# augustgw/early-exit-transformer

Hardware: AMD Instinct MI355X
Metric: mel-frames/sec encoder forward (all exits) + summed per-exit CTC loss, d_model=256 12-layer (higher is better)
Workload: dtype fp16x3 (hi/lo-split fp16 MFMA operands, three products per GEMM, fp32 accumulate; v_mfma_f32_16x16x32_f16); 1 GPU; early_conformer ctc 12-layer d_model=256 (6 exits x 2), batch 64/GPU, mel [80 x 1027] -> T'=256, log-normal synthetic mel, random-init weights (BASELINE.json configs[1]); global_batch=64, mel_frames=1027, parallelism=dp1 (utterance-batch shards), precision_mode=f16x3

## Files before the change

early_exit_transformer_amd/csrc/eec_blocks.h:

```cpp
#pragma once
#include "eec_kernels.h"

namespace eec {

constexpr int kLinThreads = 512;
template <int D>
constexpr int kLinLds = 2 * Geo<D>::kAPlane;
#ifndef EEC_LPF
#define EEC_LPF 4
#endif
constexpr int kLPF = EEC_LPF;

constexpr int kQkvStageLd = 80, kQkvStageLdV = 144, kQkvStageBytes = 64 * kQkvStageLd;
static_assert(32 * kQkvStageLdV <= kQkvStageBytes, "V^T staging fits the Q / K staging area");
constexpr int kQkvFragLd = 1056;
static_assert(4 * kQkvFragLd <= kQkvStageBytes && (kQkvFragLd / 2) % 16 == 0, "fragment-major V^T staging");
__device__ __forceinline__ int vt_perm(int t) {
  return (t & ~12) | ((t & 4) << 1) | ((t & 8) >> 1);
}

template <int MT, int NT>
__device__ __forceinline__ void acc_init_bias(f32x16 (&acc)[MT][NT], const float* __restrict__ bias_n0, float scale = 1.0f) {
  const int hh = lane_id() >> 5;
#pragma unroll
  for (int nt = 0; nt < NT; ++nt)
#pragma unroll
    for (int g = 0; g < 4; ++g) {
      const float4 bb = *(const float4*)(bias_n0 + 32 * nt + 8 * g + 4 * hh);
#pragma unroll
      for (int mt = 0; mt < MT; ++mt) {
        acc[mt][nt][4 * g + 0] = bb.x * scale;
        acc[mt][nt][4 * g + 1] = bb.y * scale;
        acc[mt][nt][4 * g + 2] = bb.z * scale;
        acc[mt][nt][4 * g + 3] = bb.w * scale;
      }
    }
}

template <int NP, int MT, int NT>
__device__ __forceinline__ void acc_init_bias_np(f32x16 (&acc)[MT][NT], const float* __restrict__ bias_n0, float scale = 1.0f) {
  if constexpr (kMfma16For<NP>) {
    const int lane = lane_id(), hh = lane >> 5, u = (lane >> 4) & 1;
#pragma unroll
    for (int nt = 0; nt < NT; ++nt)
#pragma unroll
      for (int ra = 0; ra < 2; ++ra) {
        const float4 bb = *(const float4*)(bias_n0 + 32 * nt + 16 * ra + 8 * hh + 4 * u);
#pragma unroll
        for (int mt = 0; mt < MT; ++mt)
#pragma unroll
          for (int cb = 0; cb < 2; ++cb) {
            acc[mt][nt][4 * (2 * ra + cb) + 0] = bb.x * scale;
            acc[mt][nt][4 * (2 * ra + cb) + 1] = bb.y * scale;
            acc[mt][nt][4 * (2 * ra + cb) + 2] = bb.z * scale;
            acc[mt][nt][4 * (2 * ra + cb) + 3] = bb.w * scale;
          }
      }
  } else {
    acc_init_bias<MT, NT>(acc, bias_n0, scale);
  }
}

template <int KS>
__device__ __forceinline__ const uint4* wfrag_lane(const uint4* wp, int nt) {
  return wp + (size_t)nt * KS * 128 + lane_id();
}

constexpr int kProjNWB = 2;
template <int NP, int PF, int NT>
struct ProjStream {
  WRing<(NP == 8 ? 1 : NP), PF, NT> r;
  WGroupF8<NT> wg[NP == 8 ? kProjNWB : 1];
};
struct WMat {
  const uint4* wp;
  const uint4* wf8;
};
template <int D, int NP, int PF, int NT>
__device__ __forceinline__ void proj_fill(ProjStream<NP, PF, NT>& st, const WMat& w, int t0) {
  constexpr int KS = D / 16, NG = D / 64;
  if constexpr (NP == 8) {
    const uint4* rec = w.wf8 + (size_t)t0 * NG * kF8Rec + lane_id();
    ring_fill_f8<PF, NT>(st.r, rec, (size_t)NG * kF8Rec);
#pragma unroll
    for (int g = 0; g < kProjNWB; ++g) f8_group_load<NT>(st.wg[g], rec + (size_t)g * kF8Rec, (size_t)NG * kF8Rec);
  } else {
    ring_fill<NP, PF, NT>(st.r, wfrag_lane<KS>(w.wp, t0), (size_t)KS * 128, KS);
  }
}
template <int D, int NP, int PF, int NT, int MT>
__device__ __forceinline__ void proj_gemm(f32x16 (&acc)[MT][NT], const char* smem, ProjStream<NP, PF, NT>& st, const WMat& w, int t0,
                                          int row_stride_mul = 1) {
  using G = Geo<D>;
  constexpr int KS = D / 16, NG = D / 64;
  const int lane = lane_id(), hh = lane >> 5;
  const char* a_lane = smem + (lane & 31) * G::kALd + hh * 16;
  if constexpr (NP == 8) {
    const char* a8_lane = smem + G::kAPlane + (lane & 31) * G::kA8Ld + hh * 32;
    const uint4* rec = w.wf8 + (size_t)t0 * NG * kF8Rec + lane;
    gemm_ring_f8<NG, NT, true, PF, NoSide, 0, kProjNWB, MT>(acc, a_lane, G::kALd, a8_lane, G::kA8Ld, rec,
                                                                                                    (size_t)NG * kF8Rec, st.r, st.wg);
  } else {
    gemm_ring<NP, KS, NT, true, PF, NoSide, 0, MT, !kMfma16For<NP>, true>(acc, a_lane, G::kALd, G::kAPlane, wfrag_lane<KS>(w.wp, t0), (size_t)KS * 128, st.r);
  }
  (void)row_stride_mul;
}

template <int D, int NP>
__device__ __forceinline__ void qkv_body(char* smem, const QkvArgs& a, int row0, ProjStream<NP, kLPF, Geo<D>::kNW>& rq, char* stage = nullptr) {
  using G = Geo<D>;
  constexpr int MT = G::kMT, NW = G::kNW;
  const int lane = lane_id(), w = wave_id(), hh = lane >> 5;
  const int dh = D / a.H;
  const bool fast = D == 256 && stage != nullptr && dh == 32 && a.Tq % G::kRows == 0 && a.Tp == a.Tq;
  char* const stg = stage ? stage + w * kQkvStageBytes : nullptr;
  [[maybe_unused]] auto store_rows_fast = [&](const f32x16 (&acc)[MT][NW], float scale, half_t* p_hi, half_t* p_lo, size_t off) {
    h4 lo4[MT][4];
#pragma unroll
    for (int mt = 0; mt < MT; ++mt)
#pragma unroll
      for (int g = 0; g < 4; ++g) {
        h4 o;
#pragma unroll
        for (int i = 0; i < 4; ++i) {
          const float v = acc[mt][0][4 * g + i] * scale;
          o[i] = to_half_sat(v);
          lo4[mt][g][i] = (half_t)(v - (float)o[i]);
        }
        *(h4*)(stg + (mt * 32 + (lane & 31)) * kQkvStageLd + (8 * g + 4 * hh) * 2) = o;
      }
    asm volatile("" ::: "memory");
    auto tile_out = [&](half_t* dstp) {
      if (a.vt_frag) {
#pragma unroll
        for (int k = 0; k < 4; ++k)
          *(uint4*)(dstp + off + k * 512 + lane * 8) = *(const uint4*)(stg + ((k >> 1) * 32 + (lane & 31)) * kQkvStageLd + (k & 1) * 32 + hh * 16);
      } else {
#pragma unroll
        for (int k = 0; k < 4; ++k) {
          const int row = (lane >> 2) + 16 * k;
          *(uint4*)(dstp + off + (size_t)row * 32 + (lane & 3) * 8) = *(const uint4*)(stg + row * kQkvStageLd + (lane & 3) * 16);
        }
      }
    };
    tile_out(p_hi);
    asm volatile("" ::: "memory");
    if (p_lo) {
#pragma unroll
      for (int mt = 0; mt < MT; ++mt)
#pragma unroll
        for (int g = 0; g < 4; ++g) *(h4*)(stg + (mt * 32 + (lane & 31)) * kQkvStageLd + (8 * g + 4 * hh) * 2) = lo4[mt][g];
      asm volatile("" ::: "memory");
      tile_out(p_lo);
      asm volatile("" ::: "memory");
    }
  };
  const WMat wm{a.wp, a.wf8};
  ProjStream<NP, kLPF, NW> rk;
  int rb[MT], rt[MT];
  bool ok[MT];
#pragma unroll
  for (int mt = 0; mt < MT; ++mt) {
    const int row = row0 + mt * 32 + (lane & 31);
    ok[mt] = row < a.M;
    rb[mt] = row / a.Tq;
    rt[mt] = row - rb[mt] * a.Tq;
  }
  const int t0 = NW * w;
  constexpr int TQ = D / 32;
  int hd[NW], d0[NW];
#pragma unroll
  for (int j = 0; j < NW; ++j) {
    const int n0 = 32 * (t0 + j);
    hd[j] = n0 / dh;
    d0[j] = n0 - hd[j] * dh + 4 * hh;
  }

  f32x16 acc[MT][NW];
  proj_fill<D, NP, kLPF, NW>(rk, wm, TQ + t0);
  acc_init_bias_np<NP, MT, NW>(acc, a.bias + 32 * t0);
  proj_gemm<D, NP, kLPF, NW, MT>(acc, smem, rq, wm, t0);
  proj_fill<D, NP, kLPF, NW>(rq, wm, 2 * TQ + t0);
  if (fast) {
    if constexpr (D == 256) {
      const int b0 = row0 / a.Tq, tt0 = row0 - b0 * a.Tq;
      store_rows_fast(acc, kLog2e * rsqrtf((float)dh), a.q, a.q_lo, ((size_t)(b0 * a.H + w) * a.Tp + tt0) * 32);
    }
  } else {
    const float scale = kLog2e * rsqrtf((float)dh);
#pragma unroll
    for (int mt = 0; mt < MT; ++mt)
      if (ok[mt]) {
#pragma unroll
        for (int j = 0; j < NW; ++j) {
          const size_t qoff = ((size_t)(rb[mt] * a.H + hd[j]) * a.Tp + rt[mt]) * dh + d0[j];
          half_t* dst = a.q + qoff;
#pragma unroll
          for (int g = 0; g < 4; ++g) {
            h4 o, ol;
#pragma unroll
            for (int i = 0; i < 4; ++i) {
              const float v = acc[mt][j][4 * g + i] * scale;
              o[i] = to_half_sat(v);
              ol[i] = (half_t)(v - (float)o[i]);
            }
            *(h4*)(dst + 8 * g) = o;
            if (a.q_lo) *(h4*)(a.q_lo + qoff + 8 * g) = ol;
          }
        }
      }
  }
  acc_init_bias_np<NP, MT, NW>(acc, a.bias + D + 32 * t0);
  proj_gemm<D, NP, kLPF, NW, MT>(acc, smem, rk, wm, TQ + t0);
  if (fast) {
    if constexpr (D == 256) {
      const int b0 = row0 / a.Tq, tt0 = row0 - b0 * a.Tq;
      store_rows_fast(acc, 1.0f, a.k, a.k_lo, ((size_t)(b0 * a.H + w) * a.Tp + tt0) * 32);
    }
  } else
#pragma unroll
  for (int mt = 0; mt < MT; ++mt)
    if (ok[mt]) {
#pragma unroll
      for (int j = 0; j < NW; ++j) {
        const size_t koff = ((size_t)(rb[mt] * a.H + hd[j]) * a.Tp + rt[mt]) * dh + d0[j];
        half_t* dst = a.k + koff;
#pragma unroll
        for (int g = 0; g < 4; ++g) {
          h4 o, ol;
#pragma unroll
          for (int i = 0; i < 4; ++i) {
            const float v = acc[mt][j][4 * g + i];
            o[i] = to_half_sat(v);
            ol[i] = (half_t)(v - (float)o[i]);
          }
          *(h4*)(dst + 8 * g) = o;
          if (a.k_lo) *(h4*)(a.k_lo + koff + 8 * g) = ol;
        }
      }
    }
  acc_init_bias_np<NP, MT, NW>(acc, a.bias + 2 * D + 32 * t0);
  proj_gemm<D, NP, kLPF, NW, MT>(acc, smem, rq, wm, 2 * TQ + t0);
  if (fast) {
    if constexpr (D == 256) {
      const int b0 = row0 / a.Tq, tt0 = row0 - b0 * a.Tq;
      const size_t vbase = ((size_t)(b0 * a.H + w) * 32) * a.Tp + tt0;
      const int dstride = a.vt_frag ? 16 : kQkvStageLdV;
      int sbase[MT];
#pragma unroll
      for (int mt = 0; mt < MT; ++mt) {
        const int tcol = vt_perm(mt * 32 + (lane & 31));
        sbase[mt] = a.vt_frag ? ((tcol >> 5) * 2 + ((tcol >> 4) & 1)) * kQkvFragLd + ((tcol >> 3) & 1) * (kQkvFragLd / 2) + (tcol & 7) * 2 : tcol * 2;
      }
      auto plane = [&](half_t* dstp, bool lo_plane) {
#pragma unroll
        for (int mt = 0; mt < MT; ++mt)
#pragma unroll
          for (int g = 0; g < 4; ++g)
#pragma unroll
            for (int i = 0; i < 4; ++i) {
              const float v = acc[mt][0][4 * g + i];
              const half_t hi = to_half_sat(v);
              *(half_t*)(stg + sbase[mt] + (8 * g + 4 * hh + i) * dstride) = lo_plane ? (half_t)(v - (float)hi) : hi;
            }
        asm volatile("" ::: "memory");
        if (a.vt_frag) {
          half_t* const fb = dstp + (size_t)(b0 * a.H + w) * 32 * a.Tp + (size_t)(tt0 >> 5) * 1024;
#pragma unroll
          for (int k = 0; k < 4; ++k)
            *(uint4*)(fb + k * 512 + lane * 8) = *(const uint4*)(stg + k * kQkvFragLd + (lane >> 5) * (kQkvFragLd / 2) + (lane & 31) * 16);
        } else {
#pragma unroll
          for (int k = 0; k < 4; ++k) {
            const int d = (lane >> 3) + 8 * k;
            *(uint4*)(dstp + vbase + (size_t)d * a.Tp + (lane & 7) * 8) = *(const uint4*)(stg + d * kQkvStageLdV + (lane & 7) * 16);
          }
        }
        asm volatile("" ::: "memory");
      };
      plane(a.vt, false);
      if (a.vt_lo) plane(a.vt_lo, true);
    }
  } else
#pragma unroll
  for (int mt = 0; mt < MT; ++mt)
    if (ok[mt]) {
#pragma unroll
      for (int j = 0; j < NW; ++j) {
        const size_t voff = ((size_t)(rb[mt] * a.H + hd[j]) * dh + d0[j]) * a.Tp + vt_perm(rt[mt]);
        half_t* dst = a.vt + voff;
#pragma unroll
        for (int g = 0; g < 4; ++g)
#pragma unroll
          for (int i = 0; i < 4; ++i) {
            const float v = acc[mt][j][4 * g + i];
            const half_t hi = to_half_sat(v);
            *(dst + (size_t)(8 * g + i) * a.Tp) = hi;
            if (a.vt_lo) {
              half_t* const lo = a.vt_lo + voff + (size_t)(8 * g + i) * a.Tp;
              *lo = (half_t)(v - (float)hi);
            }
          }
      }
    }
}

constexpr int kDwTaps = 31;
constexpr int kDwHalo = (kDwTaps - 1) / 2;
constexpr int kDwFrames = 16;
constexpr int kDwWin = kDwFrames + kDwTaps - 1;
constexpr int kDPF = 4;
template <int D>
struct DwGeo {
  using G = Geo<D>;
  static constexpr bool kTapsLds = D == 256;
  static constexpr int kGRows = G::kRows + kDwTaps - 1;
  static constexpr int kGLd = D * 2;
  static constexpr int kLds = 2 * G::kAPlane + kGRows * kGLd + (kTapsLds ? kDwTaps * D * 4 : 0);
  static_assert((D / 2) * (G::kRows / kDwFrames) == 512, "thread = 2 channels x 16 frames");
};

template <int D, int NP>
__device__ __forceinline__ void dw_front(char* smem, const DwArgs& d, int M, int row0) {
  using G = Geo<D>;
  using DG = DwGeo<D>;
  constexpr int kGRows = DG::kGRows, kGLd = DG::kGLd;
  char* lds_g = smem + 2 * G::kAPlane;
  float* lds_w = (float*)(lds_g + kGRows * kGLd);
  const int Tq = d.Tq;
  const int c = (threadIdx.x % (D / 2)) * 2, tg = threadIdx.x / (D / 2);
  typedef float f32x2 __attribute__((ext_vector_type(2)));
  [[maybe_unused]] f32x2 taps[DG::kTapsLds ? 1 : kDwTaps];
  {
    constexpr int PPR = D / 8;
    constexpr int GIT = (kGRows * PPR + 511) / 512, WIT = DG::kTapsLds ? (kDwTaps * D / 4 + 511) / 512 : 1;
    uint4 gv[GIT];
    [[maybe_unused]] float4 wv[WIT];
#pragma unroll
    for (int it = 0; it < GIT; ++it) {
      const int p = it * 512 + threadIdx.x, rl = p / PPR, c16 = p % PPR, row = row0 - kDwHalo + rl;
      gv[it] = make_uint4(0, 0, 0, 0);
      if (rl < kGRows && row >= 0 && row < M) gv[it] = *(const uint4*)(d.g + (size_t)row * D + c16 * 8);
    }
    if constexpr (DG::kTapsLds) {
#pragma unroll
      for (int it = 0; it < WIT; ++it) {
        const int p = it * 512 + threadIdx.x;
        wv[it] = make_float4(0.f, 0.f, 0.f, 0.f);
        if (p < kDwTaps * D / 4) wv[it] = ((const float4*)d.wfold)[p];
      }
    } else {
      static_range<0, kDwTaps>([&](auto jt) { taps[decltype(jt)::value] = *(const f32x2*)(d.wfold + decltype(jt)::value * D + c); });
    }
    __builtin_amdgcn_sched_barrier(0);
#pragma unroll
    for (int it = 0; it < GIT; ++it) {
      const int p = it * 512 + threadIdx.x, rl = p / PPR, c16 = p % PPR;
// ... 159 lines not shown
```

early_exit_transformer_amd/csrc/ffn.hip:

```cpp
#ifdef EEC_FFN_TRAIN_BWD
#define EEC_OPERAND_BF16 1
#endif
#if defined(EEC_FFN_TRAIN) || defined(EEC_FFN_TRAIN_BWD)
#define EEC_MFMA16_NP1 1
#endif
#include "eec_blocks.h"
#include "eec_drop.h"

namespace eec {

constexpr int kFfnThreads = 512;
constexpr int kFC = 128;
constexpr int kHLd = (kFC + 8) * 2;
template <int D>
struct FfnGeo {
  using G = Geo<D>;
  static constexpr int kHPlane = G::kRows * kHLd;
  static constexpr int kNT2 = D / 128;
  static constexpr int kLds = 2 * G::kAPlane + (4 * kHPlane > G::kETile ? 4 * kHPlane : G::kETile);
};
#ifndef EEC_TR_NT
#define EEC_TR_NT 1
#endif
#if defined(EEC_FFN_TRAIN_BWD) && !defined(EEC_PF1_NP3)
// ... 87 lines not shown
};

template <int D, int NPN, bool HAS_RES>
__device__ __forceinline__ void chain_rowpass(char* smem, const char* lds_e, float* __restrict__ x, RowV<Geo<D>::kQ> (&xr)[Geo<D>::kRPW],
                                              int row0, int M, float scale, const float* __restrict__ fin_g,
                                              const float* __restrict__ fin_b, float* __restrict__ tap,
                                              const float* __restrict__ nln_g, const float* __restrict__ nln_b,
                                              int lane = lane_id(), int w = wave_id()) {
  using G = Geo<D>;
  constexpr int RPW = G::kRPW, Q = G::kQ;
  RowV<Q> v[RPW];
#pragma unroll
  for (int i = 0; i < RPW; ++i) {
    v[i] = HAS_RES ? xr[i] : zero_row<Q>();
#pragma unroll
    for (int q = 0; q < Q; ++q) {
      const float4 e = *(const float4*)(lds_e + (w * RPW + i) * G::kELd + (q * 256 + lane * 4) * 4);
      v[i].p[q].x += scale * e.x;
      v[i].p[q].y += scale * e.y;
      v[i].p[q].z += scale * e.z;
      v[i].p[q].w += scale * e.w;
    }
  }
  if (fin_g) layer_norm_rows<D, RPW>(v, load_row<D>(fin_g, lane), load_row<D>(fin_b, lane));
#pragma unroll
  for (int i = 0; i < RPW; ++i) {
    const int row = row0 + w * RPW + i;
    if (row < M) {
      store_row<D>(x + (size_t)row * D, v[i], lane);
      if (tap) store_row<D>(tap + (size_t)row * D, v[i], lane);
    }
  }
  if constexpr (NPN != 0) {
    layer_norm_rows<D, RPW>(v, load_row<D>(nln_g, lane), load_row<D>(nln_b, lane));
    rows_to_planes<D, NPN, RPW>(smem, v, w * RPW, row0, M, true, lane);
  }
}

template <int D, int NP, int ACT, int FNP, int QNP, int NS, int TR = 0>
#ifndef EEC_FFN_MINWAVES
#define EEC_FFN_MINWAVES 2
#endif
__global__ __launch_bounds__(kFfnThreads, EEC_FFN_MINWAVES) void ffn_chain_kernel(ChainArgs a) {
  static_assert(!TR || (FNP == 0 && QNP == 0 && NS == 1 && ACT == 2 && NP != 8), "TR: one plain stage");
  static_assert(TR || ACT != 2, "ACT = 2 is the training variant's");
  static_assert((TR == 2) == (EEC_OPERAND_BF16 != 0), "the backward variant (and only it) runs on bf16 operands");
  using G = Geo<D>;
  using FG = FfnGeo<D>;
  constexpr int MT = G::kMT, NW = G::kNW, KS = G::kKS, RPW = G::kRPW, NT2 = FG::kNT2;
  constexpr int kALd = G::kALd, kAPlane = G::kAPlane, kA8Ld = G::kA8Ld, kHPlane = FG::kHPlane;
  constexpr size_t nts = (size_t)KS * 128;
  extern __shared__ __attribute__((aligned(16))) char smem[];
  constexpr int kPF1 = FfnPf<D, NP>::P1, kPF2 = FfnPf<D, NP>::P2;
  constexpr int NH = (NP == 8 && NT2 > 2) ? NT2 / 2 : 1, NTP = NT2 / NH;
  const int lane = lane_id(), w = wave_id();
  const int hh = lane >> 5, wl = w & 3;
  const int w_s = wave_id_sgpr();
  const int wl_s = w_s & 3;
  const bool is_producer = w < 4;
  const int row0 = row_tile_index() * G::kRows;
  const int M = a.M, F = a.F;
  float* __restrict__ x = a.x;
  char* lds_h = smem + 2 * kAPlane;
  char* lds_e = lds_h;
  const char* a_lane = smem + (lane & 31) * kALd + hh * 16;

  const int nft = F / 32;
  const int nchunk = (nft + 3) / 4;
  const int ks2_total = F / 16;
#ifndef EEC_SKEW
#define EEC_SKEW 56
#endif
#ifndef EEC_WARM_SLOTS
#define EEC_WARM_SLOTS 4
#endif
  auto phys = [&](int c) { return c >= nchunk ? c - nchunk : c; };
  const size_t w2_nt_stride = (size_t)ks2_total * 128;

#ifdef EEC_TIMELINE
  int tl_idx = 0;
#endif
  TL_STAMP();
#if EEC_SKEW > 0
  for (int i = 0; i < (int)((blockIdx.x >> 3) & 3); ++i) __builtin_amdgcn_s_sleep(EEC_SKEW);
#endif
  constexpr int RNP = NP == 8 ? 1 : NP;
  constexpr bool Q16 = kMfma16For<NP>;
  auto run = [&](auto prod_tag) {
  constexpr bool producer = decltype(prod_tag)::value;
  [[maybe_unused]] const eect::DropState ds_act(eect::Drop{TR ? a.tr.p : 0.0f, a.tr.seed, a.tr.site_act});
  WRing<RNP, kPF1, 1> r1;
  WRing<RNP, kPF2, NTP> r2;
  WGroupF8<1> wg1[kNW1];
  WGroupF8<NTP> wg2[kNW2];
  const size_t w2f8_nt = (size_t)(F / 64) * kF8Rec;
  auto w1f8_lane = [&](const WPtrs& W, int ft) { return W.w1f8 + (size_t)ft * (D / 64) * kF8Rec + lane; };
  auto w2f8_lane = [&](const WPtrs& W, int c, int h = 0) {
    return W.w2f8 + ((size_t)(NT2 * wl + NTP * h) * (F / 64) + 2 * c) * kF8Rec + lane;
  };
  auto fill1 = [&](const WPtrs& W, int ft) {
    if constexpr (NP == 8) {
      ring_fill_f8<kPF1, 1>(r1, w1f8_lane(W, ft), 0);
#pragma unroll
      for (int g = 0; g < kNW1; ++g) f8_group_load<1>(wg1[g], w1f8_lane(W, ft) + (size_t)g * kF8Rec, 0);
    } else {
      ring_fill<RNP, kPF1, 1>(r1, W.w1p + (size_t)ft * nts + lane, 0, KS);
// ... 4 lines not shown
      ring_fill_f8<kPF2, NTP>(r2, w2f8_lane(W, c), w2f8_nt);
#pragma unroll
      for (int g = 0; g < kNW2; ++g) f8_group_load<NTP>(wg2[g], w2f8_lane(W, c) + (size_t)g * kF8Rec, w2f8_nt);
    } else {
      ring_fill<RNP, kPF2, NTP>(r2, W.w2p + ((size_t)(NT2 * wl) * ks2_total + c * (kFC / 16)) * 128 + lane, w2_nt_stride,
                             min(kFC / 16, ks2_total - c * (kFC / 16)));
    }
  };
  auto start_streams = [&](const WPtrs& W) {
    if constexpr (producer) {
      if (wl < nft) fill1(W, phys(0) * 4 + wl);
    } else {
      fill2(W, phys(0));
    }
  };
#define EEC_STAGE_FIELD(si, f) ((si) == 0 ? a.st[0].f : a.st[1].f)
  auto wptrs = [&](int si) {
    return WPtrs{EEC_STAGE_FIELD(si, w1p), EEC_STAGE_FIELD(si, w2p), EEC_STAGE_FIELD(si, w1f8), EEC_STAGE_FIELD(si, w2f8)};
  };

  unsigned sink_front = 0;
  if constexpr (FNP != 0) {
    ProjStream<FNP, kDPF, NW> rp;
    proj_fill<D, FNP, kDPF, NW>(rp, WMat{a.pw2.wp, a.pw2.wf8}, NW * w);
#if EEC_WARM_SLOTS > 0
    {
      const WPtrs W0 = wptrs(0);
      const size_t wbytes = NP == 8 ? (size_t)(F / 32) * (D / 64) * kF8Rec * 16 : (size_t)F * D * 2 * (NP == 3 ? 2 : 1);
      unsigned t = 0;
#pragma unroll
      for (int j = 0; j < 2; ++j) {
        t ^= touch_share(NP == 8 ? (const void*)W0.w1f8 : (const void*)W0.w1p, wbytes, wl, j);
        t ^= touch_share(NP == 8 ? (const void*)W0.w2f8 : (const void*)W0.w2p, wbytes, wl, j);
      }
      sink_front = t;
    }
#endif
    TL_STAMP();
    dw_front<D, FNP>(smem, a.dw, M, row0);
    TL_STAMP();
    RowV<G::kQ> xr[RPW];
#pragma unroll
    for (int i = 0; i < RPW; ++i) {
      const int row = row0 + w * RPW + i;
      xr[i] = zero_row<G::kQ>();
      if (row < M) xr[i] = load_row<D>(x + (size_t)row * D, lane);
    }
    __builtin_amdgcn_sched_barrier(0);
    __syncthreads();
    TL_STAMP();
    f32x16 accp[MT][NW];
    pw2_gemm<D, FNP>(accp, smem, a.pw2, rp);
    TL_STAMP();
    start_streams(wptrs(0));
    acc_swapped_to_etile<MT, NW>(lds_e, G::kELd, accp, 32 * NW * w);
    __syncthreads();
    TL_STAMP();
    chain_rowpass<D, NP, true>(smem, lds_e, x, xr, row0, M, 1.0f, nullptr, nullptr, nullptr, a.st[0].ln_g, a.st[0].ln_b);
  } else {
    const WPtrs W0 = wptrs(0);
    if constexpr (TR == 2) {
      const eect::DropState ds_res(eect::Drop{a.tr.p, a.tr.seed, a.tr.site_res});
      const float rsc = a.st[0].res_scale;
      RowV<G::kQ> v[RPW];
#pragma unroll
      for (int i = 0; i < RPW; ++i) {
        const int row = row0 + w * RPW + i;
        v[i] = zero_row<G::kQ>();
        if (row < M) v[i] = load_row<D>(x + (size_t)row * D, lane);
      }
      __builtin_amdgcn_sched_barrier(0);
      start_streams(W0);
      if (a.tr.pl_x) {
        constexpr int Q = G::kQ;
        const RowV<Q> gam = load_row<D>(a.tr.pl_g, lane);
        RowV<Q> xh[RPW];
        float rsd[RPW], c1[RPW], c2[RPW];
        RowV<Q> dgs = zero_row<Q>(), dbs = zero_row<Q>();
#pragma unroll
        for (int i = 0; i < RPW; ++i) {
          const int row = row0 + w * RPW + i;
          const bool ok = row < M;
          const float mu = ok ? a.tr.pl_mean[row] : 0.0f;
          rsd[i] = ok ? a.tr.pl_rstd[row] : 0.0f;
          xh[i] = ok ? load_row<D>(a.tr.pl_x + (size_t)row * D, lane) : zero_row<Q>();
          c1[i] = 0.0f, c2[i] = 0.0f;
#pragma unroll
          for (int q = 0; q < Q; ++q) {
            float4& h = xh[i].p[q];
            h.x = (h.x - mu) * rsd[i], h.y = (h.y - mu) * rsd[i], h.z = (h.z - mu) * rsd[i], h.w = (h.w - mu) * rsd[i];
            const float4 ev = v[i].p[q], gq = gam.p[q];
            const float tx = ev.x * gq.x, ty = ev.y * gq.y, tz = ev.z * gq.z, tw = ev.w * gq.w;
            c1[i] += tx + ty + tz + tw;
            c2[i] += tx * h.x + ty * h.y + tz * h.z + tw * h.w;
            dgs.p[q].x += ev.x * h.x, dgs.p[q].y += ev.y * h.y, dgs.p[q].z += ev.z * h.z, dgs.p[q].w += ev.w * h.w;
            dbs.p[q].x += ev.x, dbs.p[q].y += ev.y, dbs.p[q].z += ev.z, dbs.p[q].w += ev.w;
          }
        }
        wave_sum_n<RPW>(c1);
        wave_sum_n<RPW>(c2);
#pragma unroll
        for (int i = 0; i < RPW; ++i) {
          const int row = row0 + w * RPW + i;
          const float m1 = c1[i] * (1.0f / D), m2 = c2[i] * (1.0f / D);
#pragma unroll
          for (int q = 0; q < Q; ++q) {
// ... 5 lines not shown
          }
          if (row < M) store_row<D>(x + (size_t)row * D, v[i], lane);
        }
        float* pw = a.tr.pl_part + ((size_t)blockIdx.x * 8 + w) * 2 * D;
#pragma unroll
        for (int q = 0; q < Q; ++q) {
          *(float4*)(pw + q * 256 + lane * 4) = dgs.p[q];
          *(float4*)(pw + D + q * 256 + lane * 4) = dbs.p[q];
        }
      }
#pragma unroll
      for (int i = 0; i < RPW; ++i) {
        const int row = row0 + w * RPW + i;
#pragma unroll
        for (int q = 0; q < G::kQ; ++q) {
          float m[4];
          ds_res.mul4((size_t)row * D + q * 256 + lane * 4, m);
          v[i].p[q].x *= rsc * m[0], v[i].p[q].y *= rsc * m[1], v[i].p[q].z *= rsc * m[2], v[i].p[q].w *= rsc * m[3];
        }
        if (row < M) store_row<D>(a.tr.ln + (size_t)row * D, v[i], lane);
      }
      rows_to_planes<D, NP, RPW>(smem, v, w * RPW, row0, M, false);
    } else if constexpr (TR == 1) {
      const RowV<G::kQ> lg = load_row<D>(a.st[0].ln_g, lane), lb = load_row<D>(a.st[0].ln_b, lane);
      RowV<G::kQ> v[RPW];
#pragma unroll
      for (int i = 0; i < RPW; ++i) {
        const int row = row0 + w * RPW + i;
        v[i] = zero_row<G::kQ>();
        if (row < M) v[i] = load_row<D>(x + (size_t)row * D, lane);
      }
      __builtin_amdgcn_sched_barrier(0);
      start_streams(W0);
      float mu[RPW], rs[RPW];
      layer_norm_rows<D, RPW>(v, lg, lb, mu, rs);
#pragma unroll
      for (int i = 0; i < RPW; ++i) {
        const int row = row0 + w * RPW + i;
        if (row < M) {
          store_row<D>(a.tr.ln + (size_t)row * D, v[i], lane);
          if (lane == 0) a.tr.mean[row] = mu[i], a.tr.rstd[row] = rs[i];
        }
      }
      rows_to_planes<D, NP, RPW>(smem, v, w * RPW, row0, M, true);
    } else {
      rows_f32_to_planes<D, NP, true>(smem, x, row0, M, a.st[0].ln_g, a.st[0].ln_b, [&]() { start_streams(W0); });
    }
  }
  TL_STAMP();
  __syncthreads();
  TL_STAMP();

  [[maybe_unused]] ProjStream<(QNP ? QNP : 1), kLPF, NW> rq;
  unsigned sink = 0;
  const int nslots = nchunk + 2;
  f32x16 acc2c[NH][MT][NTP];
  static_range<0, NS>([&](auto si_tag) {
    constexpr int si = decltype(si_tag)::value;
    const WPtrs W = wptrs(si);
    const float* __restrict__ b1s = EEC_STAGE_FIELD(si, b1);
    if constexpr (producer) {
      [[maybe_unused]] f32x16 preq[TR == 2 ? MT : 1];
      [[maybe_unused]] auto request_pre = [&](int hcol0) {
#pragma unroll
        for (int mt = 0; mt < MT; ++mt)
#pragma unroll
          for (int g = 0; g < 4; ++g) {
            const int frame = Q16 ? mt * 32 + 16 * (g & 1) + (lane & 15) : mt * 32 + (lane & 31);
            const int hid = Q16 ? wl * 32 + 16 * (g >> 1) + 8 * hh + 4 * ((lane >> 4) & 1) : wl * 32 + 4 * hh + g * 8;
            const int row = min(row0 + frame, M - 1);
            const f32x4 v = __builtin_nontemporal_load((const f32x4*)(a.tr.pre + (size_t)row * F + hcol0 + hid));
            preq[mt][4 * g] = v[0], preq[mt][4 * g + 1] = v[1], preq[mt][4 * g + 2] = v[2], preq[mt][4 * g + 3] = v[3];
          }
      };
      auto silu_pair = [&](const f32x16 (&acc)[MT][1], char* hb, int step, h2& keep_hi, h2& keep_lo, [[maybe_unused]] int hcol0 = 0) {
        const int mt = step >> 3, q = step & 7;
        const float u0 = acc[mt][0][2 * q], u1 = acc[mt][0][2 * q + 1];
        if constexpr (TR == 2) {
          const float x0 = preq[mt][2 * q], x1 = preq[mt][2 * q + 1];
          const float sg0 = __builtin_amdgcn_rcpf(1.0f + __builtin_amdgcn_exp2f(-kLog2e * x0));
          const float sg1 = __builtin_amdgcn_rcpf(1.0f + __builtin_amdgcn_exp2f(-kLog2e * x1));
          const float t0 = u0 * sg0 * (1.0f + x0 * (1.0f - sg0)), t1 = u1 * sg1 * (1.0f + x1 * (1.0f - sg1));
          if ((q & 1) == 0) {
            keep_hi = __builtin_bit_cast(h2, t0);
            keep_lo = __builtin_bit_cast(h2, t1);
            return;
          }
          const int g = q >> 1;
          const int frame = Q16 ? mt * 32 + 16 * (g & 1) + (lane & 15) : mt * 32 + (lane & 31);
          const int hid = Q16 ? wl * 32 + 16 * (g >> 1) + 8 * hh + 4 * ((lane >> 4) & 1) : wl * 32 + 4 * hh + g * 8;
          const int row = row0 + frame;
          const size_t idx = (size_t)row * F + hcol0 + hid;
          float m[4];
          ds_act.mul4(idx, m);
          const float d0 = __builtin_bit_cast(float, keep_hi) * m[0], d1 = __builtin_bit_cast(float, keep_lo) * m[1], d2 = t0 * m[2], d3 = t1 * m[3];
          if (row < M) tape_store4(a.tr.act + idx, d0, d1, d2, d3);
          constexpr int SNPT = NP == 1 ? 1 : 3;
          const hl2_t sa = split2<SNPT>(d0, d1), sb = split2<SNPT>(d2, d3);
          char* dst = hb + frame * kHLd + hid * 2;
          h4 hi, lo;
          hi.xy = sa.hi, hi.zw = sb.hi, lo.xy = sa.lo, lo.zw = sb.lo;
          *(h4*)dst = hi;
          if (NP == 3) *(h4*)(dst + kHPlane) = lo;
          return;
        }
        if constexpr (TR == 1) {
// ... 127 lines not shown
      }
    } else {
#pragma unroll
      for (int h = 0; h < NH; ++h) zero_acc(acc2c[h]);
#if EEC_WARM_SLOTS > 0
      unsigned warm[4] = {0u, 0u, 0u, 0u};
#endif
      for (int s = 0; s < nslots; ++s) {
#if EEC_WARM_SLOTS > 0
        if (s == nslots - EEC_WARM_SLOTS) {
          const int lane_t = fresh_lane();
          if constexpr (si + 1 < NS) {
            const WPtrs Wn = wptrs(si + 1);
            const size_t wbytes = NP == 8 ? (size_t)(F / 32) * (D / 64) * kF8Rec * 16 : (size_t)F * D * 2 * (NP == 3 ? 2 : 1);
#pragma unroll
            for (int j = 0; j < 2; ++j) {
              warm[j] = touch_share(NP == 8 ? (const void*)Wn.w1f8 : (const void*)Wn.w1p, wbytes, wl_s, j, lane_t);
              warm[2 + j] = touch_share(NP == 8 ? (const void*)Wn.w2f8 : (const void*)Wn.w2p, wbytes, wl_s, j, lane_t);
            }
          } else if constexpr (QNP != 0) {
            warm[0] = QNP == 8 ? touch_share(a.qkv.wf8, (size_t)(3 * D / 32) * (D / 64) * kF8Rec * 16, wl_s, 0, lane_t)
                               : touch_share(a.qkv.wp, (size_t)3 * D * D * 2 * (QNP == 3 ? 2 : 1), wl_s, 0, lane_t);
          }
        }
#endif
        if (s >= 2) {
          const int cl = s - 2, c = phys(cl);
          const char* h_lane = lds_h + (cl & 1) * 2 * kHPlane + (lane & 31) * kHLd + hh * 16;
          const int ks2 = min(kFC / 16, ks2_total - c * (kFC / 16));
          const uint4* w2_lane = W.w2p + ((size_t)(NT2 * wl) * ks2_total + c * (kFC / 16)) * 128 + lane;
          if constexpr (NP == 8) {
            const char* h8_lane = lds_h + (cl & 1) * 2 * kHPlane + kHPlane + (lane & 31) * kH8Ld + hh * 32;
            if constexpr (NH == 1) {
              gemm_ring_f8<2, NTP, false, kPF2, NoSide, 0, kNW2, MT>(acc2c[0], h_lane, kHLd, h8_lane, kH8Ld, w2f8_lane(W, c), w2f8_nt, r2, wg2);
            } else {
#pragma unroll
              for (int h = 0; h < NH; ++h) {
                const uint4* next = h + 1 < NH ? w2f8_lane(W, c, h + 1) : (cl + 1 < nchunk ? w2f8_lane(W, phys(cl + 1), 0) : nullptr);
                gemm_ring_f8<2, NTP, false, kPF2, NoSide, 0, kNW2, MT, true>(acc2c[h], h_lane, kHLd, h8_lane, kH8Ld, w2f8_lane(W, c, h), w2f8_nt, r2, wg2, NoSide(), next);
              }
            }
          } else if (ks2 == kFC / 16) {
            gemm_ring<RNP, kFC / 16, NTP, false, kPF2, NoSide, 0, MT, !Q16, !Q16>(acc2c[0], h_lane, kHLd, kHPlane, w2_lane, w2_nt_stride, r2);
          } else {
            gemm_plain<RNP, NTP, false, MT, !Q16, !Q16>(acc2c[0], h_lane, kHLd, kHPlane, w2_lane, w2_nt_stride, ks2);
          }
          if (NH == 1 && cl + 1 < nchunk) fill2(W, phys(cl + 1));
        }
        TL_STAMP();
        __syncthreads();
        TL_STAMP();
      }
#if EEC_WARM_SLOTS > 0
      sink ^= warm[0] ^ warm[1] ^ warm[2] ^ warm[3];
#endif
    }
    const int lane_e = fresh_lane(), w_e = w_s;
    RowV<G::kQ> xr[RPW];
#pragma unroll
    for (int i = 0; i < RPW; ++i) {
      const int row = row0 + w_e * RPW + i;
      xr[i] = zero_row<G::kQ>();
      if (TR != 2 && row < M) xr[i] = load_row<D>(x + (size_t)row * D, lane_e);
    }
    __builtin_amdgcn_sched_barrier(0);
    constexpr bool more = si + 1 < NS;
    TL_STAMP();
    if constexpr (!producer) {
      if constexpr (Q16) {
#pragma unroll
        for (int h = 0; h < NH; ++h) accs_q_to_std<MT, NTP>(acc2c[h]);
      }
#pragma unroll
      for (int h = 0; h < NH; ++h)
        acc_to_etile<MT, NTP>(lds_e, G::kELd, acc2c[h], wl_s * 32 * NT2 + h * 32 * NTP, EEC_STAGE_FIELD(si, b2), lane_e);
    }
    TL_STAMP();
    if constexpr (more) {
      start_streams(wptrs(1));
    } else if constexpr (QNP != 0) {
      proj_fill<D, QNP, kLPF, NW>(rq, WMat{a.qkv.wp, a.qkv.wf8}, NW * w);
    }
    __syncthreads();
    TL_STAMP();
    const float res_scale = EEC_STAGE_FIELD(si, res_scale);
    const float *fin_g = EEC_STAGE_FIELD(si, fin_g), *fin_b = EEC_STAGE_FIELD(si, fin_b);
    float* tap = EEC_STAGE_FIELD(si, tap);
    if constexpr (TR == 2) {
      if (a.tr.x_in) {
        constexpr int Q = G::kQ;
        const RowV<Q> gam = load_row<D>(a.st[0].ln_g, lane_e);
        RowV<Q> e[RPW], xh[RPW], dres[RPW];
        float rsd[RPW], c1[RPW], c2[RPW];
        RowV<Q> dgs = zero_row<Q>(), dbs = zero_row<Q>();
#pragma unroll
        for (int i = 0; i < RPW; ++i) {
          const int rl = w_e * RPW + i, row = row0 + rl;
          const bool ok = row < M;
          const float mu = ok ? a.tr.mean[row] : 0.0f;
          rsd[i] = ok ? a.tr.rstd[row] : 0.0f;
          xh[i] = ok ? load_row<D>(a.tr.x_in + (size_t)row * D, lane_e) : zero_row<Q>();
          dres[i] = ok ? load_row<D>(x + (size_t)row * D, lane_e) : zero_row<Q>();
          c1[i] = 0.0f, c2[i] = 0.0f;
#pragma unroll
          for (int q = 0; q < Q; ++q) {
            e[i].p[q] = *(const float4*)(lds_e + rl * G::kELd + (q * 256 + lane_e * 4) * 4);
            float4& h = xh[i].p[q];
            h.x = (h.x - mu) * rsd[i], h.y = (h.y - mu) * rsd[i], h.z = (h.z - mu) * rsd[i], h.w = (h.w - mu) * rsd[i];
            const float4 ev = e[i].p[q], gq = gam.p[q];
            const float tx = ev.x * gq.x, ty = ev.y * gq.y, tz = ev.z * gq.z, tw = ev.w * gq.w;
            c1[i] += tx + ty + tz + tw;
            c2[i] += tx * h.x + ty * h.y + tz * h.z + tw * h.w;
            dgs.p[q].x += ev.x * h.x, dgs.p[q].y += ev.y * h.y, dgs.p[q].z += ev.z * h.z, dgs.p[q].w += ev.w * h.w;
            dbs.p[q].x += ev.x, dbs.p[q].y += ev.y, dbs.p[q].z += ev.z, dbs.p[q].w += ev.w;
          }
        }
        wave_sum_n<RPW>(c1);
        wave_sum_n<RPW>(c2);
#pragma unroll
        for (int i = 0; i < RPW; ++i) {
          const int row = row0 + w_e * RPW + i;
          const float m1 = c1[i] * (1.0f / D), m2 = c2[i] * (1.0f / D);
          RowV<Q> o;
#pragma unroll
          for (int q = 0; q < Q; ++q) {
            const float4 ev = e[i].p[q], gq = gam.p[q], h = xh[i].p[q], dr = dres[i].p[q];
            o.p[q].x = rsd[i] * (ev.x * gq.x - m1 - h.x * m2) + dr.x;
            o.p[q].y = rsd[i] * (ev.y * gq.y - m1 - h.y * m2) + dr.y;
            o.p[q].z = rsd[i] * (ev.z * gq.z - m1 - h.z * m2) + dr.z;
            o.p[q].w = rsd[i] * (ev.w * gq.w - m1 - h.w * m2) + dr.w;
          }
          if (row < M) store_row<D>(x + (size_t)row * D, o, lane_e);
        }
        float* red = (float*)smem;
// ... 12 lines not shown
      } else {
#pragma unroll
        for (int i = 0; i < RPW; ++i) {
          const int row = row0 + w_e * RPW + i;
          RowV<G::kQ> v;
#pragma unroll
          for (int q = 0; q < G::kQ; ++q) v.p[q] = *(const float4*)(lds_e + (w_e * RPW + i) * G::kELd + (q * 256 + lane_e * 4) * 4);
          if (row < M) store_row<D>(a.tr.y + (size_t)row * D, v, lane_e);
        }
      }
    } else if constexpr (TR == 1) {
      const eect::DropState ds_res(eect::Drop{a.tr.p, a.tr.seed, a.tr.site_res});
      RowV<G::kQ> v[RPW];
#pragma unroll
      for (int i = 0; i < RPW; ++i) {
        const int row = row0 + w_e * RPW + i;
        v[i] = xr[i];
#pragma unroll
        for (int q = 0; q < G::kQ; ++q) {
          const float4 e = *(const float4*)(lds_e + (w_e * RPW + i) * G::kELd + (q * 256 + lane_e * 4) * 4);
          float m[4];
          ds_res.mul4((size_t)row * D + q * 256 + lane_e * 4, m);
          v[i].p[q].x += res_scale * m[0] * e.x;
          v[i].p[q].y += res_scale * m[1] * e.y;
          v[i].p[q].z += res_scale * m[2] * e.z;
          v[i].p[q].w += res_scale * m[3] * e.w;
        }
        if (row < M) store_row<D>(a.tr.y + (size_t)row * D, v[i], lane_e);
      }
      if (a.tr.ln2) {
        float mu[RPW], rs[RPW];
        layer_norm_rows<D, RPW>(v, load_row<D>(a.tr.ln2_g, lane_e), load_row<D>(a.tr.ln2_b, lane_e), mu, rs);
#pragma unroll
        for (int i = 0; i < RPW; ++i) {
          const int row = row0 + w_e * RPW + i;
          if (row < M) {
            store_row<D>(a.tr.ln2 + (size_t)row * D, v[i], lane_e);
            if (lane_e == 0) a.tr.mean2[row] = mu[i], a.tr.rstd2[row] = rs[i];
          }
        }
      }
    } else if constexpr (more) {
      chain_rowpass<D, NP, true>(smem, lds_e, x, xr, row0, M, res_scale, fin_g, fin_b, tap, a.st[1].ln_g, a.st[1].ln_b, lane_e, w_e);
    } else if constexpr (QNP != 0) {
      chain_rowpass<D, QNP, true>(smem, lds_e, x, xr, row0, M, res_scale, fin_g, fin_b, tap, a.qkv.ln_g, a.qkv.ln_b, lane_e, w_e);
    } else {
      chain_rowpass<D, 0, true>(smem, lds_e, x, xr, row0, M, res_scale, fin_g, fin_b, tap, nullptr, nullptr, lane_e, w_e);
    }
    TL_STAMP();
    if (more || QNP != 0) __syncthreads();
    TL_STAMP();
  });
  static_assert(QNP == 0 || 8 * kQkvStageBytes <= 4 * FG::kHPlane || D != 256, "qkv staging fits the H buffers");
  if constexpr (QNP != 0) qkv_body<D, QNP>(smem, a.qkv, row0, rq, D == 256 ? lds_h : nullptr);
  if ((sink ^ sink_front) == 0x9e3779b9u && M == -7) x[0] = 0.f;
  TL_STAMP();
  };
  if (is_producer)
    run(BoolTag<true>{});
  else
    run(BoolTag<false>{});
}

#if defined(EEC_TIMELINE) && (!defined(EEC_FFN_D) || EEC_FFN_D == 256)
extern "C" int eec_debug_timeline(unsigned long long* host_out, int n) {
  static unsigned long long* dev = nullptr;
  if (!dev) {
    if (hipMalloc(&dev, 8 * 2 * 128 * 8) != hipSuccess) return 1;
    (void)hipMemset(dev, 0, 8 * 2 * 128 * 8);
    (void)hipMemcpyToSymbol(HIP_SYMBOL(g_timeline), &dev, sizeof(dev));
    return 0;
  }
  (void)hipDeviceSynchronize();
  return (int)hipMemcpy(host_out, dev, (size_t)n * 8, hipMemcpyDeviceToHost);
}
#endif

template <int D, int NP, int ACT, int FNP, int QNP, int NS, int TR = 0>
static hipError_t launch_chain_t(const ChainArgs& a, hipStream_t st) {
  auto k = ffn_chain_kernel<D, NP, ACT, FNP, QNP, NS, TR>;
  constexpr int lds = FNP != 0 ? (DwGeo<D>::kLds > FfnGeo<D>::kLds ? DwGeo<D>::kLds : FfnGeo<D>::kLds) : FfnGeo<D>::kLds;
  if (hipError_t e = ensure_max_lds((const void*)k, lds); e != hipSuccess) return e;
  const int grid = (a.M + Geo<D>::kRows - 1) / Geo<D>::kRows;
  hipLaunchKernelGGL(k, dim3(grid), dim3(kFfnThreads), lds, st, a);
  return hipGetLastError();
}

#if defined(EEC_FFN_TRAIN_BWD)
hipError_t launch_ffn_train_bwd(const ChainArgs& a, int np, hipStream_t st) {
  if (a.nstage != 1 || a.F < 32 || a.F % 32 != 0 || (np != 1 && np != 3)) return hipErrorInvalidValue;
  if (!a.tr.pre || !a.tr.act || !a.tr.ln) return hipErrorInvalidValue;
  if (a.tr.x_in ? (!a.tr.mean || !a.tr.rstd || !a.tr.ln_part || !a.st[0].ln_g) : !a.tr.y) return hipErrorInvalidValue;
  if (a.tr.pl_x && (!a.tr.pl_mean || !a.tr.pl_rstd || !a.tr.pl_g || !a.tr.pl_part)) return hipErrorInvalidValue;
  if (a.D == 256) return np == 3 ? launch_chain_t<256, 3, 2, 0, 0, 1, 2>(a, st) : launch_chain_t<256, 1, 2, 0, 0, 1, 2>(a, st);
  if (a.D == 512) return np == 3 ? launch_chain_t<512, 3, 2, 0, 0, 1, 2>(a, st) : launch_chain_t<512, 1, 2, 0, 0, 1, 2>(a, st);
  return hipErrorInvalidValue;
}
}
#elif defined(EEC_FFN_TRAIN)
hipError_t launch_ffn_train_fwd(const ChainArgs& a, int np, hipStream_t st) {
  if (a.nstage != 1 || a.F < 32 || a.F % 32 != 0 || (np != 1 && np != 3)) return hipErrorInvalidValue;
  if (!a.tr.y || !a.tr.ln || !a.tr.mean || !a.tr.rstd || !a.tr.pre || !a.tr.act) return hipErrorInvalidValue;
  if (a.D == 256) return np == 3 ? launch_chain_t<256, 3, 2, 0, 0, 1, 1>(a, st) : launch_chain_t<256, 1, 2, 0, 0, 1, 1>(a, st);
  if (a.D == 512) return np == 3 ? launch_chain_t<512, 3, 2, 0, 0, 1, 1>(a, st) : launch_chain_t<512, 1, 2, 0, 0, 1, 1>(a, st);
  return hipErrorInvalidValue;
}
}
// ... 71 lines not shown
```

Baseline: 20.01 million mel-frames/s.

## Fuse Q/K/V projections into one three-tile GEMM pass in FFN tail

For d_model 256 with split-fp16 weights, each wave now computes its head's Q, K and V column tiles together in a single GEMM over the shared LDS activation tile, with its own weight ring prefetched during the preceding row pass, replacing three sequential projection GEMMs with separate ring fills. The V^T store path is factored into a reusable lambda, and bias init gains a stride parameter. Warm-slot sink values are kept alive with empty asm instead of XORed into a live register, to cut register pressure. It holds three accumulator tiles at once and uses a shallower prefetch depth, which could raise register use or expose weight-load latency.

```diff
diff --git a/early_exit_transformer_amd/csrc/eec_blocks.h b/early_exit_transformer_amd/csrc/eec_blocks.h
--- a/early_exit_transformer_amd/csrc/eec_blocks.h
+++ b/early_exit_transformer_amd/csrc/eec_blocks.h
@@ -38,14 +38,14 @@
 }
 
 template <int NP, int MT, int NT>
-__device__ __forceinline__ void acc_init_bias_np(f32x16 (&acc)[MT][NT], const float* __restrict__ bias_n0, float scale = 1.0f) {
+__device__ __forceinline__ void acc_init_bias_np(f32x16 (&acc)[MT][NT], const float* __restrict__ bias_n0, float scale = 1.0f, int nt_stride = 32) {
   if constexpr (kMfma16For<NP>) {
     const int lane = lane_id(), hh = lane >> 5, u = (lane >> 4) & 1;
 #pragma unroll
     for (int nt = 0; nt < NT; ++nt)
 #pragma unroll
       for (int ra = 0; ra < 2; ++ra) {
-        const float4 bb = *(const float4*)(bias_n0 + 32 * nt + 16 * ra + 8 * hh + 4 * u);
+        const float4 bb = *(const float4*)(bias_n0 + nt_stride * nt + 16 * ra + 8 * hh + 4 * u);
 #pragma unroll
         for (int mt = 0; mt < MT; ++mt)
 #pragma unroll
@@ -106,15 +106,27 @@
   (void)row_stride_mul;
 }
 
+template <int D>
+__device__ __forceinline__ bool qkv_fast(const QkvArgs& a, bool staged) {
+  return D == 256 && staged && D / a.H == 32 && a.Tq % Geo<D>::kRows == 0 && a.Tp == a.Tq;
+}
+constexpr int kQkvPF3 = 2;
 template <int D, int NP>
-__device__ __forceinline__ void qkv_body(char* smem, const QkvArgs& a, int row0, ProjStream<NP, kLPF, Geo<D>::kNW>& rq, char* stage = nullptr) {
+__device__ __forceinline__ void qkv_fill3(ProjStream<NP, kQkvPF3, 3>& st, const QkvArgs& a, int t0) {
+  constexpr int KS = D / 16, TQ = D / 32;
+  ring_fill<NP, kQkvPF3, 3>(st.r, wfrag_lane<KS>(a.wp, t0), (size_t)TQ * KS * 128, KS);
+}
+
+template <int D, int NP, bool P3>
+__device__ __forceinline__ void qkv_body_t(char* smem, const QkvArgs& a, int row0, ProjStream<NP, kLPF, Geo<D>::kNW>& rq, char* stage,
+                                           ProjStream<NP, kQkvPF3, 3>& rq3) {
   using G = Geo<D>;
   constexpr int MT = G::kMT, NW = G::kNW;
-  const int lane = lane_id(), w = wave_id(), hh = lane >> 5;
+  const int lane = P3 ? fresh_lane() : lane_id(), w = P3 ? wave_id_sgpr() : wave_id(), hh = lane >> 5;
   const int dh = D / a.H;
-  const bool fast = D == 256 && stage != nullptr && dh == 32 && a.Tq % G::kRows == 0 && a.Tp == a.Tq;
+  const bool fast = qkv_fast<D>(a, stage != nullptr);
   char* const stg = stage ? stage + w * kQkvStageBytes : nullptr;
-  [[maybe_unused]] auto store_rows_fast = [&](const f32x16 (&acc)[MT][NW], float scale, half_t* p_hi, half_t* p_lo, size_t off) {
+  [[maybe_unused]] auto store_rows_fast = [&](const auto& acc, const int j, float scale, half_t* p_hi, half_t* p_lo, size_t off) {
     h4 lo4[MT][4];
 #pragma unroll
     for (int mt = 0; mt < MT; ++mt)
@@ -123,7 +135,7 @@
         h4 o;
 #pragma unroll
         for (int i = 0; i < 4; ++i) {
-          const float v = acc[mt][0][4 * g + i] * scale;
+          const float v = acc[mt][j][4 * g + i] * scale;
           o[i] = to_half_sat(v);
           lo4[mt][g][i] = (half_t)(v - (float)o[i]);
         }
@@ -155,6 +167,61 @@
       asm volatile("" ::: "memory");
     }
   };
+  [[maybe_unused]] auto store_vt_fast = [&](const auto& acc, const int j) {
+    const int b0 = row0 / a.Tq, tt0 = row0 - b0 * a.Tq;
+    const size_t vbase = ((size_t)(b0 * a.H + w) * 32) * a.Tp + tt0;
+    const int dstride = a.vt_frag ? 16 : kQkvStageLdV;
+    int sbase[MT];
+#pragma unroll
+    for (int mt = 0; mt < MT; ++mt) {
+      const int tcol = vt_perm(mt * 32 + (lane & 31));
+      sbase[mt] = a.vt_frag ? ((tcol >> 5) * 2 + ((tcol >> 4) & 1)) * kQkvFragLd + ((tcol >> 3) & 1) * (kQkvFragLd / 2) + (tcol & 7) * 2 : tcol * 2;
+    }
+    auto plane = [&](half_t* dstp, bool lo_plane) {
+#pragma unroll
+      for (int mt = 0; mt < MT; ++mt)
+#pragma unroll
+        for (int g = 0; g < 4; ++g)
+#pragma unroll
+          for (int i = 0; i < 4; ++i) {
+            const float v = acc[mt][j][4 * g + i];
+            const half_t hi = to_half_sat(v);
+            *(half_t*)(stg + sbase[mt] + (8 * g + 4 * hh + i) * dstride) = lo_plane ? (half_t)(v - (float)hi) : hi;
+          }
+      asm volatile("" ::: "memory");
+      if (a.vt_frag) {
+        half_t* const fb = dstp + (size_t)(b0 * a.H + w) * 32 * a.Tp + (size_t)(tt0 >> 5) * 1024;
+#pragma unroll
+        for (int k = 0; k < 4; ++k)
+          *(uint4*)(fb + k * 512 + lane * 8) = *(const uint4*)(stg + k * kQkvFragLd + (lane >> 5) * (kQkvFragLd / 2) + (lane & 31) * 16);
+      } else {
+#pragma unroll
+        for (int k = 0; k < 4; ++k) {
+          const int d = (lane >> 3) + 8 * k;
+          *(uint4*)(dstp + vbase + (size_t)d * a.Tp + (lane & 7) * 8) = *(const uint4*)(stg + d * kQkvStageLdV + (lane & 7) * 16);
+        }
+      }
+      asm volatile("" ::: "memory");
+    };
+    plane(a.vt, false);
+    if (a.vt_lo) plane(a.vt_lo, true);
+  };
+  if constexpr (P3) {
+    static_assert(D == 256 && NP == 3, "one-pass Q / K / V: split format at d_model 256");
+    if (fast) {
+      constexpr int KS = D / 16, TQ = D / 32;
+      f32x16 acc3[MT][3];
+      acc_init_bias_np<NP, MT, 3>(acc3, a.bias + 32 * w, 1.0f, D);
+      const char* a_lane = smem + (lane & 31) * G::kALd + hh * 16;
+      gemm_ring<NP, KS, 3, true, kQkvPF3, NoSide, 0, MT, false, true>(acc3, a_lane, G::kALd, G::kAPlane, wfrag_lane<KS>(a.wp, w), (size_t)TQ * KS * 128, rq3.r);
+      const int b0 = row0 / a.Tq, tt0 = row0 - b0 * a.Tq;
+      const size_t off = ((size_t)(b0 * a.H + w) * a.Tp + tt0) * 32;
+      store_rows_fast(acc3, 0, kLog2e * rsqrtf((float)dh), a.q, a.q_lo, off);
+      store_rows_fast(acc3, 1, 1.0f, a.k, a.k_lo, off);
+      store_vt_fast(acc3, 2);
+      return;
+    }
+  }
   const WMat wm{a.wp, a.wf8};
   ProjStream<NP, kLPF, NW> rk;
   int rb[MT], rt[MT];
@@ -184,7 +251,7 @@
   if (fast) {
     if constexpr (D == 256) {
       const int b0 = row0 / a.Tq, tt0 = row0 - b0 * a.Tq;
-      store_rows_fast(acc, kLog2e * rsqrtf((float)dh), a.q, a.q_lo, ((size_t)(b0 * a.H + w) * a.Tp + tt0) * 32);
+      store_rows_fast(acc, 0, kLog2e * rsqrtf((float)dh), a.q, a.q_lo, ((size_t)(b0 * a.H + w) * a.Tp + tt0) * 32);
     }
   } else {
     const float scale = kLog2e * rsqrtf((float)dh);
@@ -215,7 +282,7 @@
   if (fast) {
     if constexpr (D == 256) {
       const int b0 = row0 / a.Tq, tt0 = row0 - b0 * a.Tq;
-      store_rows_fast(acc, 1.0f, a.k, a.k_lo, ((size_t)(b0 * a.H + w) * a.Tp + tt0) * 32);
+      store_rows_fast(acc, 0, 1.0f, a.k, a.k_lo, ((size_t)(b0 * a.H + w) * a.Tp + tt0) * 32);
     }
   } else
 #pragma unroll
@@ -242,45 +309,7 @@
   acc_init_bias_np<NP, MT, NW>(acc, a.bias + 2 * D + 32 * t0);
   proj_gemm<D, NP, kLPF, NW, MT>(acc, smem, rq, wm, 2 * TQ + t0);
   if (fast) {
-    if constexpr (D == 256) {
-      const int b0 = row0 / a.Tq, tt0 = row0 - b0 * a.Tq;
-      const size_t vbase = ((size_t)(b0 * a.H + w) * 32) * a.Tp + tt0;
-      const int dstride = a.vt_frag ? 16 : kQkvStageLdV;
-      int sbase[MT];
-#pragma unroll
-      for (int mt = 0; mt < MT; ++mt) {
-        const int tcol = vt_perm(mt * 32 + (lane & 31));
-        sbase[mt] = a.vt_frag ? ((tcol >> 5) * 2 + ((tcol >> 4) & 1)) * kQkvFragLd + ((tcol >> 3) & 1) * (kQkvFragLd / 2) + (tcol & 7) * 2 : tcol * 2;
-      }
-      auto plane = [&](half_t* dstp, bool lo_plane) {
-#pragma unroll
-        for (int mt = 0; mt < MT; ++mt)
-#pragma unroll
-          for (int g = 0; g < 4; ++g)
-#pragma unroll
-            for (int i = 0; i < 4; ++i) {
-              const float v = acc[mt][0][4 * g + i];
-              const half_t hi = to_half_sat(v);
-              *(half_t*)(stg + sbase[mt] + (8 * g + 4 * hh + i) * dstride) = lo_plane ? (half_t)(v - (float)hi) : hi;
-            }
-        asm volatile("" ::: "memory");
-        if (a.vt_frag) {
-          half_t* const fb = dstp + (size_t)(b0 * a.H + w) * 32 * a.Tp + (size_t)(tt0 >> 5) * 1024;
-#pragma unroll
-          for (int k = 0; k < 4; ++k)
-            *(uint4*)(fb + k * 512 + lane * 8) = *(const uint4*)(stg + k * kQkvFragLd + (lane >> 5) * (kQkvFragLd / 2) + (lane & 31) * 16);
-        } else {
-#pragma unroll
-          for (int k = 0; k < 4; ++k) {
-            const int d = (lane >> 3) + 8 * k;
-            *(uint4*)(dstp + vbase + (size_t)d * a.Tp + (lane & 7) * 8) = *(const uint4*)(stg + d * kQkvStageLdV + (lane & 7) * 16);
-          }
-        }
-        asm volatile("" ::: "memory");
-      };
-      plane(a.vt, false);
-      if (a.vt_lo) plane(a.vt_lo, true);
-    }
+    if constexpr (D == 256) store_vt_fast(acc, 0);
   } else
 #pragma unroll
   for (int mt = 0; mt < MT; ++mt)
@@ -303,6 +332,12 @@
           }
       }
     }
+}
+
+template <int D, int NP>
+__device__ __forceinline__ void qkv_body(char* smem, const QkvArgs& a, int row0, ProjStream<NP, kLPF, Geo<D>::kNW>& rq, char* stage = nullptr) {
+  ProjStream<NP, kQkvPF3, 3> none;
+  qkv_body_t<D, NP, false>(smem, a, row0, rq, stage, none);
 }
 
 constexpr int kDwTaps = 31;
diff --git a/early_exit_transformer_amd/csrc/ffn.hip b/early_exit_transformer_amd/csrc/ffn.hip
--- a/early_exit_transformer_amd/csrc/ffn.hip
+++ b/early_exit_transformer_amd/csrc/ffn.hip
@@ -163,6 +163,9 @@
   constexpr size_t nts = (size_t)KS * 128;
   extern __shared__ __attribute__((aligned(16))) char smem[];
   constexpr int kPF1 = FfnPf<D, NP>::P1, kPF2 = FfnPf<D, NP>::P2;
+  constexpr bool kQkv3 = D == 256 && NP == 3 && QNP == 3 && TR == 0;
+  constexpr bool kSinkEarly = kQkv3;
+  auto keep_alive = [](unsigned v) { asm volatile("" ::"v"(v)); };
   constexpr int NH = (NP == 8 && NT2 > 2) ? NT2 / 2 : 1, NTP = NT2 / NH;
   const int lane = lane_id(), w = wave_id();
   const int hh = lane >> 5, wl = w & 3;
@@ -273,6 +276,7 @@
     f32x16 accp[MT][NW];
     pw2_gemm<D, FNP>(accp, smem, a.pw2, rp);
     TL_STAMP();
+    if constexpr (kSinkEarly) keep_alive(sink_front), sink_front = 0;
     start_streams(wptrs(0));
     acc_swapped_to_etile<MT, NW>(lds_e, G::kELd, accp, 32 * NW * w);
     __syncthreads();
@@ -384,6 +388,7 @@
   TL_STAMP();
 
   [[maybe_unused]] ProjStream<(QNP ? QNP : 1), kLPF, NW> rq;
+  [[maybe_unused]] ProjStream<(QNP ? QNP : 1), kQkvPF3, 3> rq3;
   unsigned sink = 0;
   const int nslots = nchunk + 2;
   f32x16 acc2c[NH][MT][NTP];
@@ -617,7 +622,8 @@
         TL_STAMP();
       }
 #if EEC_WARM_SLOTS > 0
-      sink ^= warm[0] ^ warm[1] ^ warm[2] ^ warm[3];
+      if constexpr (kSinkEarly) keep_alive(warm[0] ^ warm[1] ^ warm[2] ^ warm[3]);
+      else sink ^= warm[0] ^ warm[1] ^ warm[2] ^ warm[3];
 #endif
     }
     const int lane_e = fresh_lane(), w_e = w_s;
@@ -644,7 +650,11 @@
     if constexpr (more) {
       start_streams(wptrs(1));
     } else if constexpr (QNP != 0) {
-      proj_fill<D, QNP, kLPF, NW>(rq, WMat{a.qkv.wp, a.qkv.wf8}, NW * w);
+      if (kQkv3 && qkv_fast<D>(a.qkv, true)) {
+        if constexpr (kQkv3) qkv_fill3<D, QNP>(rq3, a.qkv, w);
+      } else {
+        proj_fill<D, QNP, kLPF, NW>(rq, WMat{a.qkv.wp, a.qkv.wf8}, NW * w);
+      }
     }
     __syncthreads();
     TL_STAMP();
@@ -763,7 +773,7 @@
     TL_STAMP();
   });
   static_assert(QNP == 0 || 8 * kQkvStageBytes <= 4 * FG::kHPlane || D != 256, "qkv staging fits the H buffers");
-  if constexpr (QNP != 0) qkv_body<D, QNP>(smem, a.qkv, row0, rq, D == 256 ? lds_h : nullptr);
+  if constexpr (QNP != 0) qkv_body_t<D, QNP, kQkv3>(smem, a.qkv, row0, rq, D == 256 ? lds_h : nullptr, rq3);
   if ((sink ^ sink_front) == 0x9e3779b9u && M == -7) x[0] = 0.f;
   TL_STAMP();
   };
```

Measured after the change: 20.09 million mel-frames/s (median of 4 runs). No clear change (+0.4%).
